# dalek-cryptography/curve25519-dalek

Measured on AMD Instinct MI355X. Metric: MSM scalar-mults/sec (variable-base Pippenger MSM), higher is better.
Workload: dtype u32 limbs (radix 2^25.5), u64 accumulators

## Files before the change

curve25519-dalek_amd/csrc/msm.hip:

```cpp
#include <hip/hip_runtime.h>
#include <algorithm>
#include <stdio.h>
#include <stdlib.h>
#include <string.h>
#include <stdexcept>
#include <string>
#include <vector>
#include "../../include/c25519_hip.h"
#include "devio.h"
#include "sc_sha.h"
#include "sc28.h"
#include "kernels.h"
#include "ctx.h"
#include "msm_internal.h"
#include "msm_sort.h"
#include "host51.h"
#include "ffi.h"
#include "capi_util.h"
#include <functional>

using namespace c25519;

namespace c25519 {

// ... 390 lines not shown
    msm_geom g;
    msm_layout(n, g);
    *c = g.c; *nwin = g.nwin;
    for (int k = 0; k < g.nwin; k++) { pos[k] = g.pos[k]; wid[k] = g.wid[k]; }
    for (int i = 0; i < 8; i++) addk[i] = g.addk[i];
    return C25519_OK;
}

EXPORT int32_t c25519_debug_sort(c25519_ctx *ctx, const uint8_t *d_scalars, uint64_t n, uint64_t layout_terms, int32_t reps) {
    HIPCHK(hipSetDevice(ctx->device));
    if (n <= msm_small_max() || n > (1ull << 22)) return bad_arg(ctx, "debug_sort: n outside the range of a bucket-method pass");
    msm_geom g;
    msm_layout(layout_terms ? layout_terms : n, g);
    for (int i = 0; i < reps; i++) {
        msm_plan pl;
        pl.bad_sticky = nullptr;
        int32_t r = msm_enqueue_sort(ctx, d_scalars, n, g, dslot(ctx, 0), nullptr, pl);
        if (r) return r;
    }
    HIPCHK(hipStreamSynchronize(ctx->stream));
    return C25519_OK;
}

static_assert(C25519_SLOT_U32 == MSM_MAX_WIN * 40 + 16, "slot layout");

int32_t msm_enqueue_acc(c25519_ctx *ctx, const msm_plan &pl, const uint32_t *d_pts, uint32_t *d_slot, hipEvent_t *ring, hipEvent_t wait_acc, bool cont, bool reduce,
                        const uint32_t *d_bad_sticky) {
    const msm_geom &g = pl.g;
    if (pl.n > (1ull << 25)) return bad_arg(ctx, "msm: internal error (a pass of more than 2^25 records)");
    if (pl.sort_stream && pl.sort_stream != ctx->stream) {
        HIPCHK(hipEventRecord(ctx->ev_sort, pl.sort_stream));
        HIPCHK(hipStreamWaitEvent(ctx->stream, ctx->ev_sort, 0));
    }
    hipStream_t st = ctx->stream;
    if (wait_acc) HIPCHK(hipStreamWaitEvent(st, wait_acc, 0));
    HIPCHK(hipEventRecord(ctx->ev_fork, st));
    HIPCHK(hipStreamWaitEvent(ctx->aux, ctx->ev_fork, 0));
    hipLaunchKernelGGL(k_long_segments, dim3(std::min<uint32_t>(pl.max_items, 2048u)), dim3(64), 0, ctx->aux, d_pts, pl.sorted, pl.n, g, pl.items, pl.counters, pl.max_items, pl.segs);
    hipLaunchKernelGGL(k_long_combine, dim3(std::min<uint32_t>(pl.max_long, 1024u)), dim3(64), 0, ctx->aux, pl.base, g, pl.counters, pl.max_items, pl.lgids, pl.lfirst, pl.segs, pl.buckets, cont ? 1 : 0);
    if (ring) HIPCHK(hipEventRecord(ring[0], st));
    static const int coop_reduce = C25519_KNOB("REDUCE_COOP", 1);
    const int groups = (g.ngroups > 1 && reduce && !cont && coop_reduce) ? g.ngroups : 1;
    static const int reduce_main = C25519_KNOB("REDUCE_MAIN", 1);
    const bool red_main = reduce_main && ctx->solo && reduce && !cont && groups == 1 && coop_reduce && !wait_acc;
    for (int q = 0; q < groups; q++) {
        const int k0 = groups > 1 ? g.gstart[q] : 0, k1 = groups > 1 ? g.gstart[q + 1] : g.nwin;
// ... 659 lines not shown
```

curve25519-dalek_amd/csrc/msm_internal.h:

```cpp
#pragma once
#include <hip/hip_runtime.h>
#include <stdint.h>
#include <stdlib.h>
#include "ge26.h"
#include "ctx.h"

#include "knobs.h"
namespace c25519 {
constexpr int MSM_MAX_WIN = 56;
constexpr int MSM_MAX_GROUPS = 4;
struct msm_geom { int c, nwin, half, first_unsigned, bps_log2; u32 long_cap; u32 addk[8]; unsigned char pos[MSM_MAX_WIN], wid[MSM_MAX_WIN], bps[MSM_MAX_WIN];
                  unsigned char ngroups, gstart[MSM_MAX_GROUPS + 1]; };
__host__ __device__ inline int msm_group_of(const msm_geom &g, int k) { int r = 0; for (int i = 1; i < g.ngroups; i++) r += k >= (int)g.gstart[i] ? 1 : 0; return r; }
struct msm_merged { int c, K; uint64_t ns; };
constexpr u32 LONG_CAP_MIN = 192;
constexpr u32 LONG_SEG = 1024;
}
namespace c25519 {
struct long_item;
static inline int red_lb_log2(int half) {
    static const int lb_min = [] { const int v = C25519_KNOB("RED_LB_MIN", 1); return v < 1 ? 1 : (v > 3 ? 3 : v); }();
    if (half <= 512) return 3;
    int lb = lb_min;
    while ((half >> (lb + 6)) > 64) lb++;
    return lb;
}
static inline int red_nseg(int half) { const int seg = 64 << red_lb_log2(half); return (half + seg - 1) / seg; }
constexpr int REC_TERMS_LO = 8, REC_TERMS_HI = 9, REC_PASSES = 10, REC_MAGIC = 11, REC_C = 12;
constexpr u32 REC_MAGIC_VALUE = 0x52503235u;
inline uint64_t msm_small_max() { static const uint64_t v = (uint64_t)C25519_KNOB("MSM_SMALL_MAX", 6143); return v; }
inline uint64_t verify_small_max() { static const uint64_t v = (uint64_t)C25519_KNOB("VERIFY_SMALL_MAX", 4095); return v < msm_small_max() ? v : msm_small_max(); }
inline uint64_t small_upload_max_terms() { static const uint64_t v = (uint64_t)C25519_KNOB_LL("VERIFY_STAGED_MAX", 32769); return v; }
}
static inline unsigned div_up64(uint64_t a, uint64_t b) { return (unsigned)((a + b - 1) / b); }
static inline uint32_t *slot_flags(uint32_t *slot) { return slot + c25519::MSM_MAX_WIN * 40; }
static inline uint32_t *dslot(c25519_ctx *ctx, int i) { return ctx->d_slots + (size_t)i * C25519_SLOT_U32; }
static inline const uint32_t *hslot(c25519_ctx *ctx, int i) { return (const uint32_t *)ctx->h_msm + (size_t)i * C25519_SLOT_U32; }
static inline uint32_t *drec(c25519_ctx *ctx) { return dslot(ctx, C25519_MAX_SLOTS); }
struct msm_plan {
    c25519::msm_geom g; uint64_t n, nb; int nseg; uint32_t max_items, max_long;
    uint32_t *base, *sorted, *buckets, *perm, *SW, *counters, *lgids, *lfirst, *segs, *bad_ws, *bad_sticky = nullptr; c25519::long_item *items;
    hipStream_t sort_stream;
    hipEvent_t ev_partition = nullptr;
};
void msm_sort_params(uint64_t n, c25519::msm_geom &g);
void msm_slice_params(c25519::msm_geom &g);
int32_t msm_enqueue_sort(c25519_ctx *ctx, const uint8_t *d_scalars, uint64_t n_scalars, const c25519::msm_geom &g, uint32_t *d_slot, hipStream_t sort_stream, msm_plan &pl,
                         const c25519::msm_merged *md = nullptr, uint64_t n_carve = 0, hipEvent_t lists_free = nullptr, int parity = -1);
struct msm_matrix_sort_args {
    const uint8_t *d_scalars; uint64_t n_scalars, n; int nchunk; bool use_part; int SL, PART_CHUNK, pchunks;
    uint16_t *D; uint32_t *counts, *P1, *cc, *bin_base, *flags, *totals, *ord_hist;
};
int32_t msm_matrix_sort_enqueue(c25519_ctx *ctx, const c25519::msm_geom &g, const c25519::msm_merged *md, msm_plan &pl, const msm_matrix_sort_args &a, hipStream_t st);
int32_t msm_enqueue_acc(c25519_ctx *ctx, const msm_plan &pl, const uint32_t *d_pts, uint32_t *d_slot, hipEvent_t *ring, hipEvent_t wait_acc, bool cont = false, bool reduce = true,
                        const uint32_t *d_bad_sticky = nullptr);
struct mid_run;
int32_t msm_enqueue(c25519_ctx *ctx, const uint8_t *d_scalars, uint64_t n, const uint32_t *d_pts, const c25519::msm_geom &g, uint32_t *d_slot, hipEvent_t *ring,
                    hipStream_t sort_stream, hipEvent_t wait_acc = nullptr, const struct mid_run *run = nullptr);
int32_t msm_small_enqueue(c25519_ctx *ctx, const uint8_t *d_scalars, const void *d_points, int src_fmt, uint64_t n, const c25519::msm_geom &g, uint32_t *d_slot, hipStream_t st);
c25519::ge_p3 host_p40(const uint32_t *t);
c25519::ge_p3 msm_horner(const uint32_t *cols, const c25519::msm_geom &g);
int32_t slots_collect(c25519_ctx *ctx, int count);
int32_t rec_collect(c25519_ctx *ctx);
void slot_init(uint32_t *d_slot, uint64_t terms, const uint32_t *d_pre, hipStream_t st, int c);
// ... 35 lines not shown
```

curve25519-dalek_amd/csrc/msm_sort.h:

```cpp
#pragma once
#include <hip/hip_runtime.h>
#include "devio.h"
#include "msm_internal.h"

#ifndef C25519_PRIO
#define C25519_PRIO 1
#endif
#if defined(__HIP_DEVICE_COMPILE__) && C25519_PRIO
#define C25519_PRIO_CHAIN() __builtin_amdgcn_s_setprio(3)
#define C25519_PRIO_SIDE() __builtin_amdgcn_s_setprio(2)
#ifndef C25519_PRIO_LONG_LEVEL
#define C25519_PRIO_LONG_LEVEL 2
#endif
#define C25519_PRIO_LONG() __builtin_amdgcn_s_setprio(C25519_PRIO_LONG_LEVEL)
#else
#define C25519_PRIO_LONG() do { } while (0)
#define C25519_PRIO_CHAIN() do { } while (0)
#define C25519_PRIO_SIDE() do { } while (0)
#endif

namespace c25519 {

__device__ __forceinline__ int digit_of(u32 v, int k, const msm_geom &g) {
    return (k >= g.first_unsigned) ? (v <= (u32)g.half ? (int)v : 0) : (int)v - (1 << (g.wid[k] - 1));
// ... 2 lines not shown
constexpr int PART_BPS_MAX = 512;
#ifndef C25519_PART_CAP
#define C25519_PART_CAP 17408
#endif
constexpr int PART_CAP = C25519_PART_CAP;
static inline int part_chunk(int SL) { return SL <= 128 ? 16384 : 15360; }

__host__ __device__ __forceinline__ int part_entry_shift(const msm_geom &g) { return g.bps_log2 > 8 ? 32 - g.bps_log2 : 24; }
__device__ __forceinline__ bool part_entry(u32 v, int k, const msm_geom &g, int bps, u32 t, u32 &slice, u32 &entry) {
    int d = digit_of(v, k, g);
    if (d == 0) return false;
    u32 b = (u32)((d > 0 ? d : -d) - 1);
    const int sh = part_entry_shift(g);
    slice = b >> bps;
    entry = ((b & ((1u << bps) - 1u)) << sh) | (d < 0 ? (1u << (sh - 1)) : 0u) | t;
    return true;
}
__device__ __forceinline__ u32 part_entry_final(u32 ev, int sh) { return (ev & ((1u << (sh - 1)) - 1u)) | ((ev >> (sh - 1)) << 31); }

constexpr int SWEEP_TPT = 8, SWEEP_THREADS = 1024, SWEEP_WAVES = SWEEP_THREADS / 64, SWEEP_CHUNK = SWEEP_THREADS * SWEEP_TPT;
constexpr int P2G_ITER = 48;

struct long_item { u32 gid, lo, hi, first; };
__device__ __forceinline__ void order_note_bucket(u32 c, u64 G, const msm_geom &g, const u32 *__restrict__ base, u32 *h, u32 max_items, long_item *__restrict__ items,
                                                  u32 *__restrict__ counters, u32 *__restrict__ long_gids, u32 *__restrict__ long_first) {
    atomicAdd(&h[255u - (c > 255u ? 255u : c)], 1u);
    if (c > g.long_cap) {
        const int k = (int)(G / g.half), b = (int)(G % g.half);
        const u32 lo = base[(u64)k * (g.half + 1) + b], hi = lo + c;
        const u32 nseg = (c + LONG_SEG - 1) / LONG_SEG;
        const u32 first = atomicAdd(&counters[0], nseg);
        const u32 lb = atomicAdd(&counters[1], 1u);
        long_gids[lb] = (u32)G;
        long_first[lb] = first;
        for (u32 sg = 0; sg < nseg && first + sg < max_items; sg++) {
            long_item it; it.gid = (u32)G; it.lo = lo + sg * LONG_SEG; it.hi = (it.lo + LONG_SEG < hi) ? it.lo + LONG_SEG : hi; it.first = first;
            items[first + sg] = it;
        }
    }
}

}
```

curve25519-dalek_amd/csrc/msm_sort.hip:

```cpp
#include <hip/hip_runtime.h>
#include <algorithm>
#include <stdlib.h>
#include <string.h>
#include <stdexcept>
#include <string>
#include <vector>
#include <functional>
#include "../../include/c25519_hip.h"
#include "devio.h"
#include "sc_sha.h"
#include "sc28.h"
#include "kernels.h"
#include "ctx.h"
#include "msm_internal.h"
#include "msm_sort.h"
#include "ffi.h"
#include "capi_util.h"

using namespace c25519;


namespace c25519 {

struct sweep_regs { u32 s[SWEEP_TPT][8]; };
// ... 4 lines not shown
    for (int r = 0; r < SWEEP_TPT; r++) {
        const u64 t = lo + (u64)r * THREADS + threadIdx.x;
        u32 w[8] = {0, 0, 0, 0, 0, 0, 0, 0};
        if (t < n && nt) {
            const sweep_u32x4 *q = reinterpret_cast<const sweep_u32x4 *>(scalars) + 2 * t;
            const sweep_u32x4 a = __builtin_nontemporal_load(q), b = __builtin_nontemporal_load(q + 1);
            w[0] = a.x; w[1] = a.y; w[2] = a.z; w[3] = a.w; w[4] = b.x; w[5] = b.y; w[6] = b.z; w[7] = b.w;
        } else if (t < n) load8(scalars, t, w);
        if (bad_scalar && (w[7] >> 31)) atomicOr(bad_scalar, 1u);
        u32 carry = 0;
#pragma unroll
        for (int i = 0; i < 8; i++) { const u64 v = (u64)w[i] + g.addk[i] + carry; R.s[r][i] = (u32)v; carry = (u32)(v >> 32); }
    }
}
__device__ __forceinline__ u32 sweep_take(sweep_regs &R, int r, int wd) {
    const u32 v = R.s[r][0] & ((1u << wd) - 1u);
#pragma unroll
    for (int i = 0; i < 7; i++) R.s[r][i] = __funnelshift_r(R.s[r][i], R.s[r][i + 1], (u32)wd);
    R.s[r][7] >>= wd;
    return v;
}
template <int THREADS>
__global__ void __launch_bounds__(THREADS) k_sweep_local(const uint8_t *__restrict__ scalars, u64 n, msm_geom g, int SL, u32 *__restrict__ lsg, u32 *__restrict__ bad_blk,
                                                               u32 *__restrict__ P1, u64 wstride, u32 *__restrict__ zero_words, int nzero, int nt) {
    C25519_PRIO_CHAIN();
    extern __shared__ u32 sm[];
    constexpr int NW = THREADS / 64, CHUNK = THREADS * SWEEP_TPT;
    u32 *cnt = sm;
    u32 *cur = sm + NW * SL;
    u32 *ls = sm + 2 * NW * SL;
    u32 *stage = ls + SL + 1;
    __shared__ u32 wtot[NW];
    __shared__ u32 sbad;
    const int j = blockIdx.x, nchunk = gridDim.x, w = threadIdx.x >> 6, lane = threadIdx.x & 63;
    if (blockIdx.x == 0) for (int i = threadIdx.x; i < nzero; i += THREADS) zero_words[i] = 0;
    if (threadIdx.x == 0) sbad = 0;
    const int total = NW * SL, ept = total >= THREADS ? total / THREADS : 1;
    const int base = (int)threadIdx.x * ept;
    for (int i = threadIdx.x; i < total; i += THREADS) cnt[i] = 0;
    __syncthreads();
    const u64 lo = (u64)j * CHUNK;
    sweep_regs R;
    sweep_load<THREADS>(scalars, n, lo, g, R, &sbad, nt);
#pragma unroll 1
    for (int k = 0; k < g.nwin; k++) {
        const int wd = g.wid[k], bps = g.bps[k];
        u32 ent[SWEEP_TPT], slc[SWEEP_TPT];
#pragma unroll
        for (int r = 0; r < SWEEP_TPT; r++) {
            const u32 v = sweep_take(R, r, wd);
            slc[r] = 0xffffffffu;
            u32 sl, e;
            if (part_entry(v, k, g, bps, (u32)lo + (u32)r * THREADS + threadIdx.x, sl, e)) {
                slc[r] = sl * NW + ((u32)w ^ ((sl >> 2) & (NW - 1)));
                ent[r] = e;
                atomicAdd(&cnt[slc[r]], 1u);
            }
        }
        __syncthreads();
        u32 v4[4], tsum = 0;
#pragma unroll
        for (int e = 0; e < 4; e++) {
            v4[e] = 0;
            if (e < ept && base + e < total) { v4[e] = cnt[base + e]; cnt[base + e] = 0; }
            tsum += v4[e];
        }
        u32 inc = tsum;
        for (int off = 1; off < 64; off <<= 1) { const u32 x = __shfl_up(inc, off, 64); if (lane >= off) inc += x; }
        if (lane == 63) wtot[w] = inc;
        __syncthreads();
        u32 run = inc - tsum;
#pragma unroll
        for (int q = 0; q < NW; q++) run += q < w ? wtot[q] : 0u;
#pragma unroll
        for (int e = 0; e < 4; e++) {
            if (e < ept && base + e < total) {
                const int idx = base + e;
                cur[idx] = run;
                if ((idx & (NW - 1)) == 0) ls[idx / NW] = run;
                if (idx == total - 1) ls[SL] = run + v4[e];
            }
            run += v4[e];
        }
        __syncthreads();
#pragma unroll
        for (int r = 0; r < SWEEP_TPT; r++)
            if (slc[r] != 0xffffffffu) stage[atomicAdd(&cur[slc[r]], 1u)] = ent[r];
        __syncthreads();
        const u32 tot = ls[SL];
        u32 *dst = P1 + (u64)k * wstride + (u64)j * CHUNK;
        for (u32 i = threadIdx.x; i < tot; i += THREADS) dst[i] = stage[i];
        for (int i = threadIdx.x; i <= SL; i += THREADS) lsg[((u64)k * (SL + 1) + i) * nchunk + j] = ls[i];
    }
    if (threadIdx.x == 0) bad_blk[j] = sbad;
}
__global__ void __launch_bounds__(256) k_bin_totals(const u32 *__restrict__ lsg, int nchunk, int SL, int nbins, u32 *__restrict__ binm, const u32 *__restrict__ bad_blk,
                                                    u32 *__restrict__ bad_ws, u32 *__restrict__ bad_sticky) {
    C25519_PRIO_CHAIN();
    if (blockIdx.x == 0) {
        u32 any = 0;
        for (int i = threadIdx.x; i < nchunk; i += 256) any |= bad_blk[i];
        any = __syncthreads_or((int)any);
        if (threadIdx.x == 0) { *bad_ws = any ? 1u : 0u; if (any && bad_sticky) atomicOr(bad_sticky, 1u); }
    }
    const int bin = blockIdx.x * 4 + (threadIdx.x >> 6), lane = threadIdx.x & 63;
    if (bin >= nbins) return;
    const int k = bin / SL, s = bin % SL;
    const u32 *row0 = lsg + ((u64)k * (SL + 1) + s) * nchunk, *row1 = row0 + nchunk;
    u32 sum = 0;
    for (int j = lane; j < nchunk; j += 64) sum += row1[j] - row0[j];
// ... 69 lines not shown
            for (u32 o = st + lane; o < en; o += 64) atomicAdd(&cnt[src[(u64)j * chunk + o] >> sh], 1u);
        }
    }
    __syncthreads();
    if (tid < 64) {
        const int per = PART_BPS >> 6;
        u32 c4[8] = {0, 0, 0, 0, 0, 0, 0, 0}, sum = 0;
        for (int q = 0; q < per; q++) { c4[q] = cnt[per * tid + q]; sum += c4[q]; }
        u32 inc = sum;
        for (int off = 1; off < 64; off <<= 1) { u32 x = __shfl_up(inc, off, 64); if (tid >= off) inc += x; }
        u32 run = inc - sum;
        for (int q = 0; q < per; q++) { cur[per * tid + q] = run; run += c4[q]; }
    }
    __syncthreads();
    if (tid < PART_BPS) {
        const u64 b = (u64)sidx * PART_BPS + tid;
        totals[(u64)k * g.half + b] = cnt[tid];
        base[(u64)k * (g.half + 1) + b] = b0 + cur[tid];
    }
    __syncthreads();
    if (tid < PART_BPS) order_note_bucket(cnt[tid], (u64)k * g.half + (u64)sidx * PART_BPS + tid, g, base, oh, max_items, items, counters, long_gids, long_first);
    __syncthreads();
    if (tid < 256 && oh[tid]) atomicAdd(&ord_hist[256 * msm_group_of(g, k) + tid], oh[tid]);
    if (fits) {
#pragma unroll 1
        for (int t0 = 0; t0 < nslots; t0 += 8) {
            u32 ev[8];
            bool ok[8];
#pragma unroll
            for (int q = 0; q < 8; q++) {
                const u32 d = t0 + q < nslots ? wl[w * ITER + t0 + q] : 0u;
                ok[q] = (u32)lane < (d & 127u);
                ev[q] = ok[q] ? src[(d >> 7) + lane] : 0u;
            }
#pragma unroll
            for (int q = 0; q < 8; q++) if (ok[q]) out[atomicAdd(&cur[ev[q] >> sh], 1u)] = part_entry_final(ev[q], sh);
        }
        __syncthreads();
        for (u32 i = tid; i < m; i += 64 * NW) dst[i] = out[i];
    } else {
        for (int j = w; j < nchunk; j += NW) {
            const u32 st = row0[j], en = row1[j];
            for (u32 o0 = st; o0 < en; o0 += 64) {
                const u32 o = o0 + lane;
                const bool have = o < en;
                const u32 ev = have ? src[(u64)j * chunk + o] : 0u, bk = ev >> sh;
// ... 94 lines not shown
    const uint64_t entries = (uint64_t)g.nwin * nc;
    const uint32_t max_long = (uint32_t)std::min<uint64_t>(nb, entries / g.long_cap + 1);
    const uint32_t max_items = (uint32_t)(entries / LONG_SEG + max_long + 1);
    const size_t oLI = carve((size_t)max_items * sizeof(long_item)), oLG = carve((size_t)max_long * 4), oLF = carve((size_t)max_long * 4);
    const size_t oLS = carve((size_t)max_items * 160);
    const bool use_part = matrix && g.c >= 13 && n <= (1ull << 23) && n >= (1ull << 16);
    static const int small_blocks = C25519_KNOB("SORT_SMALL", 0);
    static const int sweep_threads = small_blocks ? 256 : (C25519_KNOB("SWEEP_THREADS", SWEEP_THREADS) == 512 ? 512 : SWEEP_THREADS);
    const int sweep_chunk = sweep_threads * SWEEP_TPT;
    const int SL = std::max(1, g.half >> g.bps_log2), PART_CHUNK = matrix ? part_chunk(SL) : sweep_chunk, pchunks = (int)((n + PART_CHUNK - 1) / PART_CHUNK), pchunks_c = (int)((nc + PART_CHUNK - 1) / PART_CHUNK);
    const size_t p1_words = matrix ? (size_t)g.nwin * nc : (size_t)g.nwin * pchunks_c * sweep_chunk;
    size_t oP1 = 0, oCC = 0, oBB = 0;
    if (!matrix || use_part) { oP1 = carve(p1_words * 4); oCC = carve((size_t)g.nwin * (SL + 1) * pchunks_c * 4); oBB = carve((size_t)g.nwin * (SL + 1) * 4 + (size_t)pchunks_c * 4); }
    int32_t r = ctx_reserve(ctx, ctx->tmp_d, off);
    if (r) return r;
    uint8_t *ws = (uint8_t *)ctx->tmp_d.p;
    uint32_t *base = (uint32_t *)(ws + oB), *sorted = (uint32_t *)(ws + oS), *buckets = (uint32_t *)(ws + oK);
    uint32_t *flags = (uint32_t *)(ws + oF), *totals = (uint32_t *)(ws + oT), *ord_hist = flags + 64, *perm = (uint32_t *)(ws + oPerm);
    const int ngr = g.ngroups > 1 ? g.ngroups : 1;
    uint32_t *ord_cursor = flags + 64 + 256 * ngr, *bad_ws = flags + 64 + 512 * ngr;
    const int ZERO_WORDS = 64 + 512 * ngr;
    if (ngr > 1 && (matrix || g.half < 1024)) return bad_arg(ctx, "msm: internal error (window groups outside the chunk-local sort)");
    pl.g = g; pl.n = n; pl.nb = nb; pl.nseg = nseg; pl.max_items = max_items; pl.max_long = max_long;
    pl.base = base; pl.sorted = sorted; pl.buckets = buckets; pl.perm = perm; pl.SW = (uint32_t *)(ws + oSW); pl.counters = flags + 8; pl.bad_ws = bad_ws;
    pl.items = (long_item *)(ws + oLI); pl.lgids = (uint32_t *)(ws + oLG); pl.lfirst = (uint32_t *)(ws + oLF); pl.segs = (uint32_t *)(ws + oLS);
    pl.sort_stream = sort_stream;
    hipStream_t st = sort_stream ? sort_stream : ctx->stream;
    if (matrix) {
        if (lists_free) HIPCHK(hipStreamWaitEvent(st, lists_free, 0));
        msm_matrix_sort_args a;
        a.d_scalars = d_scalars; a.n_scalars = n_scalars; a.n = n; a.nchunk = nchunk; a.use_part = use_part; a.SL = SL; a.PART_CHUNK = PART_CHUNK; a.pchunks = pchunks;
        a.D = (uint16_t *)(ws + oD); a.counts = (uint32_t *)(ws + oC); a.P1 = (uint32_t *)(ws + oP1); a.cc = (uint32_t *)(ws + oCC); a.bin_base = (uint32_t *)(ws + oBB);
        a.flags = flags; a.totals = totals; a.ord_hist = ord_hist;
        return msm_matrix_sort_enqueue(ctx, g, md, pl, a, st);
    }
    uint32_t *P1 = (uint32_t *)(ws + oP1), *lsg = (uint32_t *)(ws + oCC), *binm = (uint32_t *)(ws + oBB), *bad_blk = binm + (size_t)g.nwin * (SL + 1);
    const uint64_t wstride = (uint64_t)pchunks_c * sweep_chunk;
    constexpr int ITER_SMALL = 160;
    const int nw1 = sweep_chunk / SWEEP_TPT / 64;
    const size_t lds1 = ((size_t)2 * nw1 * SL + SL + 1 + sweep_chunk) * 4;
    const size_t lds2 = ((size_t)3 * PART_BPS_MAX + PART_CAP + (small_blocks ? 8 * ITER_SMALL : 16 * P2G_ITER)) * 4;
    static const int sweep_nt = C25519_KNOB("SWEEP_NT", 0);
    if (small_blocks) {
        HIPCHK(hipFuncSetAttribute(reinterpret_cast<const void *>(k_sweep_local<256>), hipFuncAttributeMaxDynamicSharedMemorySize, (int)lds1));
        HIPCHK(hipFuncSetAttribute(reinterpret_cast<const void *>(k_part2g<8, ITER_SMALL>), hipFuncAttributeMaxDynamicSharedMemorySize, (int)lds2));
        hipLaunchKernelGGL(k_sweep_local<256>, dim3(pchunks), dim3(256), lds1, st, d_scalars, n, g, SL, lsg, bad_blk, P1, wstride, flags, ZERO_WORDS, sweep_nt);
    } else if (sweep_threads == 512) {
        HIPCHK(hipFuncSetAttribute(reinterpret_cast<const void *>(k_part2g<16, P2G_ITER>), hipFuncAttributeMaxDynamicSharedMemorySize, (int)lds2));
        hipLaunchKernelGGL(k_sweep_local<512>, dim3(pchunks), dim3(512), lds1, st, d_scalars, n, g, SL, lsg, bad_blk, P1, wstride, flags, ZERO_WORDS, sweep_nt);
    } else {
        HIPCHK(hipFuncSetAttribute(reinterpret_cast<const void *>(k_sweep_local<SWEEP_THREADS>), hipFuncAttributeMaxDynamicSharedMemorySize, (int)lds1));
        HIPCHK(hipFuncSetAttribute(reinterpret_cast<const void *>(k_part2g<16, P2G_ITER>), hipFuncAttributeMaxDynamicSharedMemorySize, (int)lds2));
        hipLaunchKernelGGL(k_sweep_local<SWEEP_THREADS>, dim3(pchunks), dim3(SWEEP_THREADS), lds1, st, d_scalars, n, g, SL, lsg, bad_blk, P1, wstride, flags, ZERO_WORDS, sweep_nt);
    }
    hipLaunchKernelGGL(k_bin_totals, dim3((g.nwin * SL + 3) / 4), dim3(256), 0, st, lsg, pchunks, SL, g.nwin * SL, binm, bad_blk, bad_ws, pl.bad_sticky);
    if (pl.ev_partition) HIPCHK(hipEventRecord(pl.ev_partition, st));
    if (lists_free) HIPCHK(hipStreamWaitEvent(st, lists_free, 0));
    if (small_blocks) hipLaunchKernelGGL((k_part2g<8, ITER_SMALL>), dim3(g.nwin, SL), dim3(512), lds2, st, P1, n, wstride, (u32)sweep_chunk, g, SL, pchunks, lsg, binm, totals, base, sorted, ord_hist, max_items, pl.items, pl.counters, pl.lgids, pl.lfirst);
    else hipLaunchKernelGGL((k_part2g<16, P2G_ITER>), dim3(g.nwin, SL), dim3(1024), lds2, st, P1, n, wstride, (u32)sweep_chunk, g, SL, pchunks, lsg, binm, totals, base, sorted, ord_hist, max_items, pl.items, pl.counters, pl.lgids, pl.lfirst);
    hipLaunchKernelGGL(k_order_place<1024>, dim3(div_up64(nb, 1024)), dim3(1024), 0, st, totals, nb, ord_hist, ord_cursor, perm, g);
    HIPCHK(hipGetLastError());
    return C25519_OK;
}
```

curve25519-dalek_amd/engine.py:

```python
import ctypes as C
import os

import numpy as np

OK, NONE, SCALAR_FORMAT, VERIFY, ARRAY_LENGTH, PREHASHED_CONTEXT_LENGTH = 0, 1, 2, 3, 4, 5
DOMAIN_SEPARATOR_LENGTH = 6
H2C_NU, H2C_RO = 0, 1
LIZARD_NONE, LIZARD_OK, LIZARD_BAD_ENCODING = 0, 1, 2
MONTGOMERY_MAX_BITS = 512
FMT_EDWARDS_Y, FMT_RISTRETTO, FMT_RAW160 = 0, 1, 2
POINT_DECODES, POINT_SMALL_ORDER, POINT_TORSION_FREE = 1, 2, 4
Z_TRANSCRIPT, Z_DEVICE = 0, 1
FLAG_VARTIME_TABLES = 0x100

_HERE = os.path.dirname(os.path.abspath(__file__))
_LIB = None


class EngineError(RuntimeError):
    pass


_LIB_OVERRIDE = None

# ... 2 lines not shown
    return _LIB_OVERRIDE or os.path.join(_HERE, "lib", "libc25519hip.so")


def select_library(path):
    global _LIB_OVERRIDE
    path = os.path.abspath(path)
    if _LIB is not None and os.path.abspath(lib_path()) != path:
        raise EngineError("select_library(%s): %s is already loaded in this process" % (path, lib_path()))
    _LIB_OVERRIDE = path


_vp, _u64, _i32 = C.c_void_p, C.c_uint64, C.c_int32
_SIGS = {
    "c25519_ctx_create": (_vp, [C.c_int, C.c_uint32]),
    "c25519_ctx_destroy": (None, [_vp]),
    "c25519_ctx_set_stream": (_i32, [_vp, _vp]),
    "c25519_ctx_synchronize": (_i32, [_vp]),
    "c25519_last_error": (C.c_char_p, [_vp]),
    "c25519_last_kernel_ms": (C.c_float, [_vp]),
    "c25519_phase_ms": (C.c_float, [_vp, C.c_uint32, C.c_int]),
    "c25519_last_call_phase_ms": (C.c_float, [_vp, C.c_int, _vp]),
    "c25519_debug_batch_zs": (_i32, [_vp, _vp, _vp, _vp, _vp, _u64, C.c_uint32, _vp]),
    "c25519_debug_sort": (_i32, [_vp, _vp, _u64, _u64, C.c_int32]),
    "c25519_mul_base_batch_dev": (_i32, [_vp, _vp, _u64, C.c_int, _vp]),
    "c25519_mul_base_batch": (_i32, [_vp, _vp, _u64, C.c_int, _vp]),
    "c25519_mul_base_batch_vartime_dev": (_i32, [_vp, _vp, _u64, C.c_int, _vp]),
    "c25519_mul_base_clamped_batch_dev": (_i32, [_vp, _vp, _u64, C.c_int, _vp]),
    "c25519_mul_base_clamped_batch": (_i32, [_vp, _vp, _u64, C.c_int, _vp]),
    "c25519_basetable_create": (_vp, [_vp, _vp, C.c_int]),
    "c25519_basetable_destroy": (None, [_vp, _vp]),
    "c25519_mul_table_batch_dev": (_i32, [_vp, _vp, _vp, _u64, C.c_int, _vp]),
    "c25519_mul_table_batch": (_i32, [_vp, _vp, _vp, _u64, C.c_int, _vp]),
    "c25519_x25519_contributory_batch_dev": (_i32, [_vp, _vp, _vp, _u64, _vp, _vp]),
    "c25519_x25519_contributory_batch": (_i32, [_vp, _vp, _vp, _u64, _vp, _vp]),
    "c25519_mul_clamped_batch_dev": (_i32, [_vp, _vp, _vp, _u64, C.c_int, C.c_int, _vp, _vp]),
    "c25519_mul_clamped_batch": (_i32, [_vp, _vp, _vp, _u64, C.c_int, C.c_int, _vp, _vp]),
    "c25519_point_order_checks_batch_dev": (_i32, [_vp, _vp, _u64, C.c_int, C.c_int, _vp]),
    "c25519_point_order_checks_batch": (_i32, [_vp, _vp, _u64, C.c_int, C.c_int, _vp]),
    "c25519_host_alloc": (_vp, [C.c_size_t]),
    "c25519_host_free": (None, [_vp]),
    "c25519_last_ffi_ms": (C.c_double, [_vp, _vp, _vp]),
    "c25519_ctx_trim": (_i32, [_vp]),
    "c25519_last_kernel_name": (C.c_char_p, [_vp, C.c_int]),
    "c25519_x25519_batch_dev": (_i32, [_vp, _vp, _vp, _u64, _vp]),
    "c25519_x25519_batch": (_i32, [_vp, _vp, _vp, _u64, _vp]),
    "c25519_x25519_base_batch_dev": (_i32, [_vp, _vp, _u64, _vp]),
# ... 908 lines not shown
```

include/c25519_hip.h:

```cpp
#ifndef C25519_HIP_H
#define C25519_HIP_H
#include <stddef.h>
#include <stdint.h>

#ifdef __cplusplus
extern "C" {
#endif

#define C25519_OK 0
#define C25519_NONE 1
#define C25519_SCALAR_FORMAT 2
#define C25519_VERIFY 3
#define C25519_ARRAY_LENGTH 4
#define C25519_PREHASHED_CONTEXT_LENGTH 5
#define C25519_DOMAIN_SEPARATOR_LENGTH 6

#define C25519_FMT_EDWARDS_Y 0
#define C25519_FMT_RISTRETTO 1
#define C25519_FMT_RAW160 2

#define C25519_Z_TRANSCRIPT 0
#define C25519_Z_DEVICE 1

#define C25519_FLAG_VARTIME_TABLES 0x100u
// ... 59 lines not shown

int32_t ed25519_verify_batch_dev(c25519_ctx *ctx, const uint8_t *d_msgs, const uint64_t *d_msg_off, uint64_t msgs_len,
                                 const uint8_t *d_sigs, const uint8_t *d_pks, uint64_t n, uint32_t z_mode);
int32_t ed25519_verify_batch(c25519_ctx *ctx, const uint8_t *msgs, const uint64_t *msg_off,
                             const uint8_t *sigs, const uint8_t *pks, uint64_t n, uint32_t z_mode);
int32_t ed25519_verify_batch_multi(c25519_ctx **ctxs, int32_t nctx, const uint8_t *msgs, const uint64_t *msg_off, const uint8_t *sigs, const uint8_t *pks,
                                   uint64_t n, uint32_t z_mode);
int32_t ed25519_verify_batch_keys_dev(c25519_ctx *ctx, const uint8_t *d_msgs, const uint64_t *d_msg_off, uint64_t msgs_len,
                                      const uint8_t *d_sigs, const uint8_t *d_pks, const uint8_t *d_pk_points, uint64_t n, uint32_t z_mode);
int32_t ed25519_verify_batch_keys(c25519_ctx *ctx, const uint8_t *msgs, const uint64_t *msg_off,
                                  const uint8_t *sigs, const uint8_t *pks, const uint8_t *pk_points, uint64_t n, uint32_t z_mode);

int32_t ed25519_batch_hram_dev(c25519_ctx *ctx, const uint8_t *d_msgs, const uint64_t *d_msg_off, uint64_t msgs_len, const uint8_t *d_sigs, const uint8_t *d_pks, uint64_t n,
                               uint8_t *d_hram);
int32_t ed25519_batch_transcript_zs(const uint8_t *hram, const uint8_t *sigs, uint64_t n, uint8_t *z16);
int32_t ed25519_verify_batch_record_dev(c25519_ctx *ctx, const uint8_t *d_sigs, const uint8_t *d_pks, const uint8_t *d_pk_points, const uint8_t *d_hram, const uint8_t *d_z16,
                                        uint64_t n, uint8_t *d_record);
int32_t ed25519_fold_verify_records(c25519_ctx *ctx, const uint8_t *records, uint64_t count);

int32_t c25519_debug_batch_zs(c25519_ctx *ctx, const uint8_t *msgs, const uint64_t *msg_off, const uint8_t *sigs, const uint8_t *pks, uint64_t n,
                              uint32_t z_mode, uint8_t *out_z16);

int32_t c25519_debug_sort(c25519_ctx *ctx, const uint8_t *d_scalars, uint64_t n, uint64_t layout_terms, int32_t reps);

int32_t c25519_mul_batch_dev(c25519_ctx *ctx, const uint8_t *d_scalars, const uint8_t *d_points, uint64_t n, int in_fmt, int out_fmt, uint8_t *d_out, uint8_t *d_ok);
int32_t c25519_mul_batch(c25519_ctx *ctx, const uint8_t *scalars, const uint8_t *points, uint64_t n, int in_fmt, int out_fmt, uint8_t *out, uint8_t *ok);

int32_t c25519_mul_clamped_batch_dev(c25519_ctx *ctx, const uint8_t *d_bytes, const uint8_t *d_points, uint64_t n, int in_fmt, int out_fmt, uint8_t *d_out, uint8_t *d_ok);
int32_t c25519_mul_clamped_batch(c25519_ctx *ctx, const uint8_t *bytes, const uint8_t *points, uint64_t n, int in_fmt, int out_fmt, uint8_t *out, uint8_t *ok);

#define C25519_POINT_DECODES 1
#define C25519_POINT_SMALL_ORDER 2
#define C25519_POINT_TORSION_FREE 4
int32_t c25519_point_order_checks_batch_dev(c25519_ctx *ctx, const uint8_t *d_points, uint64_t n, int in_fmt, int which, uint8_t *d_flags);
int32_t c25519_point_order_checks_batch(c25519_ctx *ctx, const uint8_t *points, uint64_t n, int in_fmt, int which, uint8_t *flags);

int32_t c25519_double_base_batch_dev(c25519_ctx *ctx, const uint8_t *d_a, const uint8_t *d_A, const uint8_t *d_b, uint64_t n, int in_fmt, int out_fmt, uint8_t *d_out, uint8_t *d_ok);
int32_t c25519_double_base_batch(c25519_ctx *ctx, const uint8_t *a, const uint8_t *A, const uint8_t *b, uint64_t n, int in_fmt, int out_fmt, uint8_t *out, uint8_t *ok);

int32_t ed25519_verify_each_dev(c25519_ctx *ctx, const uint8_t *d_msgs, const uint64_t *d_msg_off, uint64_t msgs_len,
                                const uint8_t *d_sigs, const uint8_t *d_pks, uint64_t n, int strict, uint8_t *d_status);
int32_t ed25519_verify_each(c25519_ctx *ctx, const uint8_t *msgs, const uint64_t *msg_off, const uint8_t *sigs, const uint8_t *pks,
                            uint64_t n, int strict, uint8_t *status);

int32_t ed25519_verify_each_prehashed_dev(c25519_ctx *ctx, const uint8_t *d_prehashes, const uint8_t *context, uint32_t context_len,
                                          const uint8_t *d_sigs, const uint8_t *d_pks, uint64_t n, int strict, uint8_t *d_status);
// ... 72 lines not shown
```

Before: 1.292 billion.

## Fold bucket totals and order placement into partition kernels, rank in sweep

```diff
diff --git a/curve25519-dalek_amd/csrc/msm.hip b/curve25519-dalek_amd/csrc/msm.hip
--- a/curve25519-dalek_amd/csrc/msm.hip
+++ b/curve25519-dalek_amd/csrc/msm.hip
@@ -436,6 +436,27 @@
     return C25519_OK;
 }
 
+EXPORT int32_t c25519_debug_sort_dump(c25519_ctx *ctx, const uint8_t *d_scalars, uint64_t n, uint64_t layout_terms, uint64_t n_carve, uint32_t *dims,
+                                      uint32_t *h_base, uint32_t *h_totals, uint32_t *h_perm, uint32_t *h_sorted) {
+    HIPCHK(hipSetDevice(ctx->device));
+    if (n <= msm_small_max() || n > (1ull << 22) || (n_carve && n_carve < n)) return bad_arg(ctx, "debug_sort_dump: n outside the range of a bucket-method pass");
+    msm_geom g;
+    msm_layout(layout_terms ? layout_terms : n, g);
+    dims[0] = (uint32_t)g.nwin; dims[1] = (uint32_t)g.half; dims[2] = (uint32_t)n; dims[3] = 0;
+    if (!h_base && !h_totals && !h_perm && !h_sorted) return C25519_OK;
+    msm_plan pl;
+    pl.bad_sticky = nullptr;
+    int32_t r = msm_enqueue_sort(ctx, d_scalars, n, g, dslot(ctx, 0), nullptr, pl, nullptr, n_carve);
+    if (r) return r;
+    const size_t nb = (size_t)g.nwin * g.half;
+    if (h_base) HIPCHK(hipMemcpyAsync(h_base, pl.base, (size_t)g.nwin * (g.half + 1) * 4, hipMemcpyDeviceToHost, ctx->stream));
+    if (h_totals) HIPCHK(hipMemcpyAsync(h_totals, pl.totals, nb * 4, hipMemcpyDeviceToHost, ctx->stream));
+    if (h_perm) HIPCHK(hipMemcpyAsync(h_perm, pl.perm, nb * 4, hipMemcpyDeviceToHost, ctx->stream));
+    if (h_sorted) HIPCHK(hipMemcpyAsync(h_sorted, pl.sorted, (size_t)g.nwin * n * 4, hipMemcpyDeviceToHost, ctx->stream));
+    HIPCHK(hipStreamSynchronize(ctx->stream));
+    return C25519_OK;
+}
+
 static_assert(C25519_SLOT_U32 == MSM_MAX_WIN * 40 + 16, "slot layout");
 
 int32_t msm_enqueue_acc(c25519_ctx *ctx, const msm_plan &pl, const uint32_t *d_pts, uint32_t *d_slot, hipEvent_t *ring, hipEvent_t wait_acc, bool cont, bool reduce,
diff --git a/curve25519-dalek_amd/csrc/msm_internal.h b/curve25519-dalek_amd/csrc/msm_internal.h
--- a/curve25519-dalek_amd/csrc/msm_internal.h
+++ b/curve25519-dalek_amd/csrc/msm_internal.h
@@ -40,6 +40,7 @@
 struct msm_plan {
     c25519::msm_geom g; uint64_t n, nb; int nseg; uint32_t max_items, max_long;
     uint32_t *base, *sorted, *buckets, *perm, *SW, *counters, *lgids, *lfirst, *segs, *bad_ws, *bad_sticky = nullptr; c25519::long_item *items;
+    uint32_t *totals = nullptr;
     hipStream_t sort_stream;
     hipEvent_t ev_partition = nullptr;
 };
diff --git a/curve25519-dalek_amd/csrc/msm_sort.h b/curve25519-dalek_amd/csrc/msm_sort.h
--- a/curve25519-dalek_amd/csrc/msm_sort.h
+++ b/curve25519-dalek_amd/csrc/msm_sort.h
@@ -48,9 +48,9 @@
 constexpr int P2G_ITER = 48;
 
 struct long_item { u32 gid, lo, hi, first; };
-__device__ __forceinline__ void order_note_bucket(u32 c, u64 G, const msm_geom &g, const u32 *__restrict__ base, u32 *h, u32 max_items, long_item *__restrict__ items,
-                                                  u32 *__restrict__ counters, u32 *__restrict__ long_gids, u32 *__restrict__ long_first) {
-    atomicAdd(&h[255u - (c > 255u ? 255u : c)], 1u);
+__device__ __forceinline__ u32 order_class(u32 c) { return 255u - (c > 255u ? 255u : c); }
+__device__ __forceinline__ void order_note_long(u32 c, u64 G, const msm_geom &g, const u32 *__restrict__ base, u32 max_items, long_item *__restrict__ items,
+                                                u32 *__restrict__ counters, u32 *__restrict__ long_gids, u32 *__restrict__ long_first) {
     if (c > g.long_cap) {
         const int k = (int)(G / g.half), b = (int)(G % g.half);
         const u32 lo = base[(u64)k * (g.half + 1) + b], hi = lo + c;
@@ -65,5 +65,10 @@
         }
     }
 }
+__device__ __forceinline__ void order_note_bucket(u32 c, u64 G, const msm_geom &g, const u32 *__restrict__ base, u32 *h, u32 max_items, long_item *__restrict__ items,
+                                                  u32 *__restrict__ counters, u32 *__restrict__ long_gids, u32 *__restrict__ long_first) {
+    atomicAdd(&h[order_class(c)], 1u);
+    order_note_long(c, G, g, base, max_items, items, counters, long_gids, long_first);
+}
 
 }
diff --git a/curve25519-dalek_amd/csrc/msm_sort.hip b/curve25519-dalek_amd/csrc/msm_sort.hip
--- a/curve25519-dalek_amd/csrc/msm_sort.hip
+++ b/curve25519-dalek_amd/csrc/msm_sort.hip
@@ -50,7 +50,7 @@
 }
 template <int THREADS>
 __global__ void __launch_bounds__(THREADS) k_sweep_local(const uint8_t *__restrict__ scalars, u64 n, msm_geom g, int SL, u32 *__restrict__ lsg, u32 *__restrict__ bad_blk,
-                                                               u32 *__restrict__ P1, u64 wstride, u32 *__restrict__ zero_words, int nzero, int nt) {
+                                                               u32 *__restrict__ P1, u64 wstride, u32 *__restrict__ zero_words, int nzero, int nt, int rank) {
     C25519_PRIO_CHAIN();
     extern __shared__ u32 sm[];
     constexpr int NW = THREADS / 64, CHUNK = THREADS * SWEEP_TPT;
@@ -80,9 +80,10 @@
             slc[r] = 0xffffffffu;
             u32 sl, e;
             if (part_entry(v, k, g, bps, (u32)lo + (u32)r * THREADS + threadIdx.x, sl, e)) {
-                slc[r] = sl * NW + ((u32)w ^ ((sl >> 2) & (NW - 1)));
+                const u32 c = sl * NW + ((u32)w ^ ((sl >> 2) & (NW - 1)));
                 ent[r] = e;
-                atomicAdd(&cnt[slc[r]], 1u);
+                if (rank) slc[r] = c | atomicAdd(&cnt[c], 1u) << 16;
+                else { slc[r] = c; atomicAdd(&cnt[c], 1u); }
             }
         }
         __syncthreads();
@@ -111,9 +112,15 @@
             run += v4[e];
         }
         __syncthreads();
-#pragma unroll
-        for (int r = 0; r < SWEEP_TPT; r++)
-            if (slc[r] != 0xffffffffu) stage[atomicAdd(&cur[slc[r]], 1u)] = ent[r];
+        if (rank) {
+#pragma unroll
+            for (int r = 0; r < SWEEP_TPT; r++)
+                if (slc[r] != 0xffffffffu) stage[cur[slc[r] & 0xffffu] + (slc[r] >> 16)] = ent[r];
+        } else {
+#pragma unroll
+            for (int r = 0; r < SWEEP_TPT; r++)
+                if (slc[r] != 0xffffffffu) stage[atomicAdd(&cur[slc[r]], 1u)] = ent[r];
+        }
         __syncthreads();
         const u32 tot = ls[SL];
         u32 *dst = P1 + (u64)k * wstride + (u64)j * CHUNK;
@@ -229,6 +236,183 @@
     if (tid < PART_BPS) order_note_bucket(cnt[tid], (u64)k * g.half + (u64)sidx * PART_BPS + tid, g, base, oh, max_items, items, counters, long_gids, long_first);
     __syncthreads();
     if (tid < 256 && oh[tid]) atomicAdd(&ord_hist[256 * msm_group_of(g, k) + tid], oh[tid]);
+    if (fits) {
+#pragma unroll 1
+        for (int t0 = 0; t0 < nslots; t0 += 8) {
+            u32 ev[8];
+            bool ok[8];
+#pragma unroll
+            for (int q = 0; q < 8; q++) {
+                const u32 d = t0 + q < nslots ? wl[w * ITER + t0 + q] : 0u;
+                ok[q] = (u32)lane < (d & 127u);
+                ev[q] = ok[q] ? src[(d >> 7) + lane] : 0u;
+            }
+#pragma unroll
+            for (int q = 0; q < 8; q++) if (ok[q]) out[atomicAdd(&cur[ev[q] >> sh], 1u)] = part_entry_final(ev[q], sh);
+        }
+        __syncthreads();
+        for (u32 i = tid; i < m; i += 64 * NW) dst[i] = out[i];
+    } else {
+        for (int j = w; j < nchunk; j += NW) {
+            const u32 st = row0[j], en = row1[j];
+            for (u32 o0 = st; o0 < en; o0 += 64) {
+                const u32 o = o0 + lane;
+                const bool have = o < en;
+                const u32 ev = have ? src[(u64)j * chunk + o] : 0u, bk = ev >> sh;
+                const u32 lead_bk = __shfl(bk, __ffsll((long long)__ballot(have)) - 1, 64);
+                const unsigned long long same = __ballot(have && bk == lead_bk);
+                u32 pos = 0;
+                if (have && bk == lead_bk) {
+                    const int leader = __ffsll((long long)same) - 1;
+                    u32 first = 0;
+                    if (lane == leader) first = atomicAdd(&cur[bk], (u32)__popcll(same));
+                    first = __shfl(first, leader, 64);
+                    pos = first + (u32)__popcll(same & ((1ull << lane) - 1ull));
+                } else if (have) {
+                    pos = atomicAdd(&cur[bk], 1u);
+                }
+                if (have) dst[pos] = part_entry_final(ev, sh);
+            }
+        }
+    }
+}
+
+template <int NW, int ITER>
+__device__ __forceinline__ int p2_pieces(const u32 *__restrict__ row0, const u32 *__restrict__ row1, int nchunk, u32 chunk, int w, int lane, u32 *wl, u32 &m) {
+    int nslots = 0;
+    for (int j0 = 0; j0 < nchunk; j0 += NW * 64) {
+        const int j = j0 + w + NW * lane;
+        u32 st = 0, len = 0;
+        if (j < nchunk) { st = row0[j]; len = row1[j] - st; }
+        m += len;
+        const u32 np = (len + 63u) >> 6;
+        u32 inc = np;
+        for (int off = 1; off < 64; off <<= 1) { const u32 x = __shfl_up(inc, off, 64); if (lane >= off) inc += x; }
+        const u32 first = (u32)nslots + inc - np;
+        for (u32 p = 0; p < np; p++)
+            if (first + p < (u32)ITER) wl[w * ITER + first + p] = (((u32)j * chunk + st + 64u * p) << 7) | (len - 64u * p < 64u ? len - 64u * p : 64u);
+        nslots += (int)__shfl(inc, 63, 64);
+    }
+    return nslots;
+}
+template <int NW, int ITER>
+__global__ void __launch_bounds__(64 * NW) __attribute__((amdgpu_waves_per_eu(NW / 2, NW / 2)))
+k_part2c(const u32 *__restrict__ P1, u64 wstride, u32 chunk, msm_geom g, int SL, int nchunk, const u32 *__restrict__ lsg, u32 *__restrict__ binm,
+         const u32 *__restrict__ bad_blk, u32 *__restrict__ bad_ws, u32 *__restrict__ bad_sticky, u32 *__restrict__ totals, u32 *__restrict__ ord_hist) {
+    C25519_PRIO_CHAIN();
+    __shared__ u32 cnt[PART_BPS_MAX], oh[256], wl[NW * ITER], red[NW];
+    const int k = blockIdx.x, sidx = blockIdx.y, tid = threadIdx.x, lane = tid & 63, w = tid >> 6;
+    const int PART_BPS = 1 << g.bps[k], sh = part_entry_shift(g), grp = msm_group_of(g, k);
+    if (k == 0 && sidx == 0) {
+        u32 any = 0;
+        for (int i = tid; i < nchunk; i += 64 * NW) any |= bad_blk[i];
+        any = __syncthreads_or((int)any);
+        if (tid == 0) { *bad_ws = any ? 1u : 0u; if (any && bad_sticky) atomicOr(bad_sticky, 1u); }
+    }
+    const u32 *row0 = lsg + ((u64)k * (SL + 1) + sidx) * nchunk, *row1 = row0 + nchunk;
+    const u32 *src = P1 + (u64)k * wstride;
+    if (tid < PART_BPS) cnt[tid] = 0;
+    if (tid < 256) oh[tid] = 0;
+    u32 m = 0;
+    const int nslots = p2_pieces<NW, ITER>(row0, row1, nchunk, chunk, w, lane, wl, m);
+#pragma unroll
+    for (int d = 32; d > 0; d >>= 1) m += (u32)__shfl_xor((int)m, d, 64);
+    if (lane == 0) red[w] = m;
+    const bool fits = !__syncthreads_or(nslots > ITER);
+    if (fits) {
+#pragma unroll 1
+        for (int t0 = 0; t0 < nslots; t0 += 8) {
+            u32 ev[8];
+            bool ok[8];
+#pragma unroll
+            for (int q = 0; q < 8; q++) {
+                const u32 d = t0 + q < nslots ? wl[w * ITER + t0 + q] : 0u;
+                ok[q] = (u32)lane < (d & 127u);
+                ev[q] = ok[q] ? src[(d >> 7) + lane] : 0u;
+            }
+#pragma unroll
+            for (int q = 0; q < 8; q++) if (ok[q]) atomicAdd(&cnt[ev[q] >> sh], 1u);
+        }
+    } else {
+        for (int j = w; j < nchunk; j += NW) {
+            const u32 st = row0[j], en = row1[j];
+            for (u32 o = st + lane; o < en; o += 64) atomicAdd(&cnt[src[(u64)j * chunk + o] >> sh], 1u);
+        }
+    }
+    __syncthreads();
+    if (tid == 0) { u32 t = 0; for (int q = 0; q < NW; q++) t += red[q]; binm[(u64)k * SL + sidx] = t; }
+    if (tid < PART_BPS) {
+        const u32 c = cnt[tid];
+        totals[(u64)k * g.half + (u64)sidx * PART_BPS + tid] = c;
+        atomicAdd(&oh[order_class(c)], 1u);
+    }
+    {
+        const int per = (1 << g.bps_log2) - PART_BPS, first = (SL << g.bps[k]) + sidx * per;
+        for (int i = tid; i < per; i += 64 * NW) totals[(u64)k * g.half + first + i] = 0;
+        if (per > 0 && tid == 0) atomicAdd(&oh[255], (u32)per);
+    }
+    __syncthreads();
+    if (tid < 256 && oh[tid]) atomicAdd(&ord_hist[256 * grp + tid], oh[tid]);
+}
+template <int NW, int ITER>
+__global__ void __launch_bounds__(64 * NW) __attribute__((amdgpu_waves_per_eu(NW / 2, NW / 2)))
+k_part2p(const u32 *__restrict__ P1, u64 n, u64 wstride, u32 chunk, msm_geom g, int SL, int nchunk, const u32 *__restrict__ lsg, const u32 *__restrict__ binm,
+         const u32 *__restrict__ totals, u32 *__restrict__ base, u32 *__restrict__ sorted, const u32 *__restrict__ ord_hist, u32 *__restrict__ ord_cursor, u32 *__restrict__ perm,
+         u32 max_items, long_item *__restrict__ items, u32 *__restrict__ counters, u32 *__restrict__ long_gids, u32 *__restrict__ long_first) {
+    C25519_PRIO_CHAIN();
+    extern __shared__ u32 sm[];
+    u32 *cnt = sm, *cur = sm + PART_BPS_MAX, *oh = sm + 2 * PART_BPS_MAX, *out = sm + 3 * PART_BPS_MAX, *wl = out + PART_CAP;
+    __shared__ u32 red[NW], red_all[NW], ostart[256], owt[4];
+    const int k = blockIdx.x, sidx = blockIdx.y, tid = threadIdx.x, lane = tid & 63, w = tid >> 6;
+    const int PART_BPS = 1 << g.bps[k], sh = part_entry_shift(g), grp = msm_group_of(g, k);
+    const int per = (1 << g.bps_log2) - PART_BPS, ufirst = (SL << g.bps[k]) + sidx * per;
+    const u32 *row0 = lsg + ((u64)k * (SL + 1) + sidx) * nchunk, *row1 = row0 + nchunk;
+    const u32 *src = P1 + (u64)k * wstride;
+    const u32 mine = tid < SL ? binm[(u64)k * SL + tid] : 0u;
+    u32 part = tid < sidx ? mine : 0u, all = mine;
+    const u32 m = binm[(u64)k * SL + sidx];
+    const u64 gid = tid < PART_BPS ? (u64)k * g.half + (u64)sidx * PART_BPS + tid : (u64)k * g.half + ufirst + (tid - PART_BPS);
+    const bool item = tid < PART_BPS + per;
+    const u32 c = tid < PART_BPS ? totals[gid] : 0u;
+    const u32 hv = tid < 256 ? ord_hist[256 * grp + tid] : 0u;
+    if (tid < PART_BPS) cnt[tid] = c;
+    if (tid < 256) oh[tid] = 0;
+    u32 ign = 0;
+    const int nslots = p2_pieces<NW, ITER>(row0, row1, nchunk, chunk, w, lane, wl, ign);
+    (void)ign;
+#pragma unroll
+    for (int d = 32; d > 0; d >>= 1) { part += (u32)__shfl_xor((int)part, d, 64); all += (u32)__shfl_xor((int)all, d, 64); }
+    if (lane == 0) { red[w] = part; red_all[w] = all; }
+    u32 hinc = hv;
+    if (tid < 256) {
+        for (int off = 1; off < 64; off <<= 1) { const u32 y = __shfl_up(hinc, off, 64); if (lane >= off) hinc += y; }
+        if (lane == 63) owt[w] = hinc;
+    }
+    const bool fits = !__syncthreads_or(nslots > ITER) && m <= (u32)PART_CAP;
+    u32 b0 = 0, wtot = 0;
+#pragma unroll
+    for (int q = 0; q < NW; q++) { b0 += red[q]; wtot += red_all[q]; }
+    if (tid < 256) { u32 wb = 0; for (int q = 0; q < w; q++) wb += owt[q]; ostart[tid] = wb + hinc - hv; }
+    if (sidx == SL - 1 && tid == 0) base[(u64)k * (g.half + 1) + g.half] = wtot;
+    for (int i = tid; i < per; i += 64 * NW) base[(u64)k * (g.half + 1) + ufirst + i] = wtot;
+    u32 cls = 0, local = 0;
+    if (item) { cls = order_class(c); local = atomicAdd(&oh[cls], 1u); }
+    if (tid < 64) {
+        const int pl = PART_BPS >> 6;
+        u32 c4[8] = {0, 0, 0, 0, 0, 0, 0, 0}, sum = 0;
+        for (int q = 0; q < pl; q++) { c4[q] = cnt[pl * tid + q]; sum += c4[q]; }
+        u32 inc = sum;
+        for (int off = 1; off < 64; off <<= 1) { u32 x = __shfl_up(inc, off, 64); if (tid >= off) inc += x; }
+        u32 run = inc - sum;
+        for (int q = 0; q < pl; q++) { cur[pl * tid + q] = run; run += c4[q]; }
+    }
+    __syncthreads();
+    if (tid < 256 && oh[tid]) oh[tid] = ostart[tid] + atomicAdd(&ord_cursor[256 * grp + tid], oh[tid]);
+    if (tid < PART_BPS) base[(u64)k * (g.half + 1) + (u64)sidx * PART_BPS + tid] = b0 + cur[tid];
+    __syncthreads();
+    if (item) perm[(u64)g.gstart[grp] * g.half + oh[cls] + local] = (u32)gid;
+    if (tid < PART_BPS) order_note_long(c, gid, g, base, max_items, items, counters, long_gids, long_first);
+    u32 *dst = sorted + (u64)k * n + b0;
     if (fits) {
 #pragma unroll 1
         for (int t0 = 0; t0 < nslots; t0 += 8) {
@@ -369,7 +553,7 @@
     const int ZERO_WORDS = 64 + 512 * ngr;
     if (ngr > 1 && (matrix || g.half < 1024)) return bad_arg(ctx, "msm: internal error (window groups outside the chunk-local sort)");
     pl.g = g; pl.n = n; pl.nb = nb; pl.nseg = nseg; pl.max_items = max_items; pl.max_long = max_long;
-    pl.base = base; pl.sorted = sorted; pl.buckets = buckets; pl.perm = perm; pl.SW = (uint32_t *)(ws + oSW); pl.counters = flags + 8; pl.bad_ws = bad_ws;
+    pl.base = base; pl.totals = totals; pl.sorted = sorted; pl.buckets = buckets; pl.perm = perm; pl.SW = (uint32_t *)(ws + oSW); pl.counters = flags + 8; pl.bad_ws = bad_ws;
     pl.items = (long_item *)(ws + oLI); pl.lgids = (uint32_t *)(ws + oLG); pl.lfirst = (uint32_t *)(ws + oLF); pl.segs = (uint32_t *)(ws + oLS);
     pl.sort_stream = sort_stream;
     hipStream_t st = sort_stream ? sort_stream : ctx->stream;
@@ -388,21 +572,31 @@
     const size_t lds1 = ((size_t)2 * nw1 * SL + SL + 1 + sweep_chunk) * 4;
     const size_t lds2 = ((size_t)3 * PART_BPS_MAX + PART_CAP + (small_blocks ? 8 * ITER_SMALL : 16 * P2G_ITER)) * 4;
     static const int sweep_nt = C25519_KNOB("SWEEP_NT", 0);
+    static const int sweep_rank = C25519_KNOB("SWEEP_RANK", 1), fold = C25519_KNOB("SORT_FOLD", 1);
     if (small_blocks) {
         HIPCHK(hipFuncSetAttribute(reinterpret_cast<const void *>(k_sweep_local<256>), hipFuncAttributeMaxDynamicSharedMemorySize, (int)lds1));
-        HIPCHK(hipFuncSetAttribute(reinterpret_cast<const void *>(k_part2g<8, ITER_SMALL>), hipFuncAttributeMaxDynamicSharedMemorySize, (int)lds2));
-        hipLaunchKernelGGL(k_sweep_local<256>, dim3(pchunks), dim3(256), lds1, st, d_scalars, n, g, SL, lsg, bad_blk, P1, wstride, flags, ZERO_WORDS, sweep_nt);
+        HIPCHK(hipFuncSetAttribute(fold ? reinterpret_cast<const void *>(k_part2p<8, ITER_SMALL>) : reinterpret_cast<const void *>(k_part2g<8, ITER_SMALL>), hipFuncAttributeMaxDynamicSharedMemorySize, (int)lds2));
+        hipLaunchKernelGGL(k_sweep_local<256>, dim3(pchunks), dim3(256), lds1, st, d_scalars, n, g, SL, lsg, bad_blk, P1, wstride, flags, ZERO_WORDS, sweep_nt, sweep_rank);
     } else if (sweep_threads == 512) {
-        HIPCHK(hipFuncSetAttribute(reinterpret_cast<const void *>(k_part2g<16, P2G_ITER>), hipFuncAttributeMaxDynamicSharedMemorySize, (int)lds2));
-        hipLaunchKernelGGL(k_sweep_local<512>, dim3(pchunks), dim3(512), lds1, st, d_scalars, n, g, SL, lsg, bad_blk, P1, wstride, flags, ZERO_WORDS, sweep_nt);
+        HIPCHK(hipFuncSetAttribute(fold ? reinterpret_cast<const void *>(k_part2p<16, P2G_ITER>) : reinterpret_cast<const void *>(k_part2g<16, P2G_ITER>), hipFuncAttributeMaxDynamicSharedMemorySize, (int)lds2));
+        hipLaunchKernelGGL(k_sweep_local<512>, dim3(pchunks), dim3(512), lds1, st, d_scalars, n, g, SL, lsg, bad_blk, P1, wstride, flags, ZERO_WORDS, sweep_nt, sweep_rank);
     } else {
         HIPCHK(hipFuncSetAttribute(reinterpret_cast<const void *>(k_sweep_local<SWEEP_THREADS>), hipFuncAttributeMaxDynamicSharedMemorySize, (int)lds1));
-        HIPCHK(hipFuncSetAttribute(reinterpret_cast<const void *>(k_part2g<16, P2G_ITER>), hipFuncAttributeMaxDynamicSharedMemorySize, (int)lds2));
-        hipLaunchKernelGGL(k_sweep_local<SWEEP_THREADS>, dim3(pchunks), dim3(SWEEP_THREADS), lds1, st, d_scalars, n, g, SL, lsg, bad_blk, P1, wstride, flags, ZERO_WORDS, sweep_nt);
-    }
-    hipLaunchKernelGGL(k_bin_totals, dim3((g.nwin * SL + 3) / 4), dim3(256), 0, st, lsg, pchunks, SL, g.nwin * SL, binm, bad_blk, bad_ws, pl.bad_sticky);
+        HIPCHK(hipFuncSetAttribute(fold ? reinterpret_cast<const void *>(k_part2p<16, P2G_ITER>) : reinterpret_cast<const void *>(k_part2g<16, P2G_ITER>), hipFuncAttributeMaxDynamicSharedMemorySize, (int)lds2));
+        hipLaunchKernelGGL(k_sweep_local<SWEEP_THREADS>, dim3(pchunks), dim3(SWEEP_THREADS), lds1, st, d_scalars, n, g, SL, lsg, bad_blk, P1, wstride, flags, ZERO_WORDS, sweep_nt, sweep_rank);
+    }
+    if (fold) {
+        if (small_blocks) hipLaunchKernelGGL((k_part2c<8, ITER_SMALL>), dim3(g.nwin, SL), dim3(512), 0, st, P1, wstride, (u32)sweep_chunk, g, SL, pchunks, lsg, binm, bad_blk, bad_ws, pl.bad_sticky, totals, ord_hist);
+        else hipLaunchKernelGGL((k_part2c<16, P2G_ITER>), dim3(g.nwin, SL), dim3(1024), 0, st, P1, wstride, (u32)sweep_chunk, g, SL, pchunks, lsg, binm, bad_blk, bad_ws, pl.bad_sticky, totals, ord_hist);
+    } else hipLaunchKernelGGL(k_bin_totals, dim3((g.nwin * SL + 3) / 4), dim3(256), 0, st, lsg, pchunks, SL, g.nwin * SL, binm, bad_blk, bad_ws, pl.bad_sticky);
     if (pl.ev_partition) HIPCHK(hipEventRecord(pl.ev_partition, st));
     if (lists_free) HIPCHK(hipStreamWaitEvent(st, lists_free, 0));
+    if (fold) {
+        if (small_blocks) hipLaunchKernelGGL((k_part2p<8, ITER_SMALL>), dim3(g.nwin, SL), dim3(512), lds2, st, P1, n, wstride, (u32)sweep_chunk, g, SL, pchunks, lsg, binm, totals, base, sorted, ord_hist, ord_cursor, perm, max_items, pl.items, pl.counters, pl.lgids, pl.lfirst);
+        else hipLaunchKernelGGL((k_part2p<16, P2G_ITER>), dim3(g.nwin, SL), dim3(1024), lds2, st, P1, n, wstride, (u32)sweep_chunk, g, SL, pchunks, lsg, binm, totals, base, sorted, ord_hist, ord_cursor, perm, max_items, pl.items, pl.counters, pl.lgids, pl.lfirst);
+        HIPCHK(hipGetLastError());
+        return C25519_OK;
+    }
     if (small_blocks) hipLaunchKernelGGL((k_part2g<8, ITER_SMALL>), dim3(g.nwin, SL), dim3(512), lds2, st, P1, n, wstride, (u32)sweep_chunk, g, SL, pchunks, lsg, binm, totals, base, sorted, ord_hist, max_items, pl.items, pl.counters, pl.lgids, pl.lfirst);
     else hipLaunchKernelGGL((k_part2g<16, P2G_ITER>), dim3(g.nwin, SL), dim3(1024), lds2, st, P1, n, wstride, (u32)sweep_chunk, g, SL, pchunks, lsg, binm, totals, base, sorted, ord_hist, max_items, pl.items, pl.counters, pl.lgids, pl.lfirst);
     hipLaunchKernelGGL(k_order_place<1024>, dim3(div_up64(nb, 1024)), dim3(1024), 0, st, totals, nb, ord_hist, ord_cursor, perm, g);
diff --git a/curve25519-dalek_amd/engine.py b/curve25519-dalek_amd/engine.py
--- a/curve25519-dalek_amd/engine.py
+++ b/curve25519-dalek_amd/engine.py
@@ -48,6 +48,7 @@
     "c25519_last_call_phase_ms": (C.c_float, [_vp, C.c_int, _vp]),
     "c25519_debug_batch_zs": (_i32, [_vp, _vp, _vp, _vp, _vp, _u64, C.c_uint32, _vp]),
     "c25519_debug_sort": (_i32, [_vp, _vp, _u64, _u64, C.c_int32]),
+    "c25519_debug_sort_dump": (_i32, [_vp, _vp, _u64, _u64, _u64, _vp, _vp, _vp, _vp, _vp]),
     "c25519_mul_base_batch_dev": (_i32, [_vp, _vp, _u64, C.c_int, _vp]),
     "c25519_mul_base_batch": (_i32, [_vp, _vp, _u64, C.c_int, _vp]),
     "c25519_mul_base_batch_vartime_dev": (_i32, [_vp, _vp, _u64, C.c_int, _vp]),
diff --git a/include/c25519_hip.h b/include/c25519_hip.h
--- a/include/c25519_hip.h
+++ b/include/c25519_hip.h
@@ -105,6 +105,8 @@
                               uint32_t z_mode, uint8_t *out_z16);
 
 int32_t c25519_debug_sort(c25519_ctx *ctx, const uint8_t *d_scalars, uint64_t n, uint64_t layout_terms, int32_t reps);
+int32_t c25519_debug_sort_dump(c25519_ctx *ctx, const uint8_t *d_scalars, uint64_t n, uint64_t layout_terms, uint64_t n_carve, uint32_t *dims,
+                              uint32_t *h_base, uint32_t *h_totals, uint32_t *h_perm, uint32_t *h_sorted);
 
 int32_t c25519_mul_batch_dev(c25519_ctx *ctx, const uint8_t *d_scalars, const uint8_t *d_points, uint64_t n, int in_fmt, int out_fmt, uint8_t *d_out, uint8_t *d_ok);
 int32_t c25519_mul_batch(c25519_ctx *ctx, const uint8_t *scalars, const uint8_t *points, uint64_t n, int in_fmt, int out_fmt, uint8_t *out, uint8_t *ok);
```

Result: no change. 1.289 billion (median of 6 runs) (-0.3%).
